# verdurin/pbdagcon

Measured on AMD Instinct MI355X. Metric: consensus bases/sec (whole node), higher is better.
Workload: dtype u8

## Files before the change

### pbdagcon_amd/csrc/k_build.hip.h

```cpp
#pragma once
#include <hip/hip_runtime.h>
#include "dagcon_dev.h"
#include "k_norm_run.hip.h"

#define DG_WAVE 64
#ifndef DG_LPW
#define DG_LPW 8u
#endif

__device__ __forceinline__ bool dg_failed(const DgParams &p) {
    return __hip_atomic_load(&p.st->err_flags, __ATOMIC_RELAXED, __HIP_MEMORY_SCOPE_AGENT) != 0;
}
__device__ __forceinline__ void dg_fail(const DgParams &p, uint32_t bit) {
    atomicOr(&p.st->err_flags, bit);
}
__device__ __forceinline__ void dg_fail_target(const DgParams &p, uint32_t t, uint32_t bit) {
    atomicOr(&p.tfail[t], bit);
}
__device__ __forceinline__ bool dg_tskip(const DgParams &p, uint32_t t) {
    return !p.tactive[t] || __hip_atomic_load(&p.tfail[t], __ATOMIC_RELAXED, __HIP_MEMORY_SCOPE_AGENT) != 0;
}
__device__ __forceinline__ bool dg_askip(const DgParams &p, uint32_t a) {
    return !(p.flags & DG_F_A1_ONLY) && __hip_atomic_load(&p.tfail[p.aln_tgt[a]], __ATOMIC_RELAXED, __HIP_MEMORY_SCOPE_AGENT) != 0;
}
__device__ __forceinline__ void dg_fail_aln(const DgParams &p, uint32_t a, uint32_t bit) {
    if (p.flags & DG_F_A1_ONLY) dg_fail(p, bit);
    else dg_fail_target(p, p.aln_tgt[a], bit);
    p.st->bad_aln = a;
}

#define DG_NW 64u
#define DG_NW_BIG 512u
#define DG_REDO 0xFFFFFFFFu

template <typename CT>
__device__ __forceinline__ void dg_store_run(const DgParams &p, CT *cell, const uint32_t run) {
    if constexpr (sizeof(CT) == 1) {
        if (run > 255u) { dg_fail(p, DG_E_RUN_WIDE); return; }
    }
    *cell = (CT)run;
}

template <typename CT>
__device__ inline void dg_finish_alignment(const DgParams &p, uint32_t a, uint16_t *buf, uint32_t m) {
    const uint32_t trim = p.trim;
    uint32_t lbases = 0, rbases = 0, lo = 0, hi = m;
    uint32_t start = p.aln_start[a];
    while (lbases < trim && lo < m) {
        if (DG_T(buf[lo++]) != DG_GAP) lbases++;
    }
    while (rbases < trim && hi > lo) {
        if (DG_T(buf[--hi]) != DG_GAP) rbases++;
    }
    start += lbases;
    const bool graph = !(p.flags & DG_F_A1_ONLY);
    uint32_t t_idx = 0, r = 0;
    CT *Cm = nullptr;
    if (graph) {
        t_idx = p.aln_tgt[a];
        if (p.tactive[t_idx]) {
            const uint64_t ab = p.aln_begin[t_idx];
            r = (uint32_t)(a - ab);
            Cm = static_cast<CT *>(p.matC) + p.matc_base[t_idx] + (uint64_t)r * p.matc_stride[t_idx];
        }
    }
    const uint32_t tlen = graph ? p.tlen[t_idx] : 0xFFFFFFFFu;
    uint32_t n_ins = 0, n_del = 0, adv = 0, run = 0;
    bool conf = start >= 1;
    uint32_t i = lo;
#define DG_FIN_COL(c, ci_)                                                                \
    do {                                                                                  \
        const uint8_t qb_ = DG_Q(c), tb_ = DG_T(c);                                       \
        if (qb_ == tb_ || qb_ == DG_GAP) {                                                \
            if (Cm && conf && ((start + adv) & ((1u << p.emit_shift) - 1u)) == 0 && start + adv <= tlen + 1) \
                ck[(start + adv) >> p.emit_shift] = ci_ - run;                            \
            if (run) { if (Cm && conf && start + adv <= tlen + 1) dg_store_run(p, Cm + (start + adv), run); run = 0; } \
            adv++; n_del += (qb_ != tb_);                                                 \
            if ((uint64_t)start - 1 + adv > (uint64_t)tlen) conf = false;                 \
        } else if (tb_ == DG_GAP) { n_ins++; run++; }                                     \
    } while (0)
    uint32_t *ck = p.ckpt + p.ck_base[a];
    while (i < hi && (i & 7u)) { const uint16_t c = buf[i]; DG_FIN_COL(c, i); i++; }
    while (i + 8 <= hi) {
        const uint4 v = *reinterpret_cast<const uint4 *>(buf + i);
        const uint32_t w4[4] = {v.x, v.y, v.z, v.w};
#pragma unroll
        for (int k = 0; k < 4; k++) {
            const uint16_t c0 = (uint16_t)(w4[k] & 0xffffu), c1 = (uint16_t)(w4[k] >> 16);
            DG_FIN_COL(c0, i + 2 * k);
            DG_FIN_COL(c1, i + 2 * k + 1);
        }
        i += 8;
    }
    while (i < hi) { const uint16_t c = buf[i]; DG_FIN_COL(c, i); i++; }
    if (run && Cm && conf && ((start + adv) & ((1u << p.emit_shift) - 1u)) == 0 && start + adv <= tlen + 1)
        ck[(start + adv) >> p.emit_shift] = hi - run;
    if (run && Cm && conf && start + adv <= tlen + 1) dg_store_run(p, Cm + (start + adv), run);
#undef DG_FIN_COL
    p.n_lo[a] = lo; p.n_hi[a] = hi; p.n_start[a] = start;
    p.n_ins[a] = n_ins; p.n_del[a] = n_del;
    atomicAdd(&p.st->n_columns, (unsigned long long)(hi - lo));
    if (graph && hi > lo && !conf) dg_fail_aln(p, a, DG_E_NONCONF);
}

template <uint32_t NW, uint32_t LANES, bool RETRY>
__global__ __launch_bounds__(LANES, RETRY ? 1 : 5) void k_norm_chunk(DgParams p) {
    __shared__ uint16_t s_win[LANES * (NW + 2u)];
    const uint32_t g = threadIdx.x * gridDim.x + blockIdx.x;
    if (g >= p.n_chunks) return;
    if (dg_failed(p)) return;
    if (RETRY && p.ch_flag[g] != 2u) return;
    const uint32_t a = p.ch_aln[g];
    if (dg_askip(p, a)) { if (!RETRY) p.ch_flag[g] = 0; return; }
    const uint32_t c = g - p.ch_base[a], nwin = p.ch_base[a + 1] - p.ch_base[a];
    const uint64_t off = p.aln_off[a];
    const uint32_t len = p.aln_len[a];
    const uint8_t *q = p.q + off, *t = p.t + off;
    uint32_t flag = 0;
    DgChunkRun r;
    r.w = 0; r.tb = 0; r.dirty = false; r.overflow = false; r.badchar = false;
    uint32_t k0 = DG_CH_NONE, cn = c + 1;
    uint64_t src = 0;
    if (p.flags & DG_F_RAW) {
        if (c == 0) { k0 = 0; cn = nwin; flag = 1; }
    } else {
        k0 = dg_chunk_start(q, t, len, c);
        if (k0 != DG_CH_NONE) {
            uint16_t *win = s_win + threadIdx.x * (NW + 2u);
            src = (2ull * (off + k0) + 8ull * g + 7ull) & ~7ull;
            for (;;) {
                uint32_t k1 = len;
                for (; cn < nwin; cn++) {
                    const uint32_t s = dg_chunk_start(q, t, len, cn);
                    if (s != DG_CH_NONE) { k1 = s; break; }
                }
                if constexpr (NW == DG_NW) r = dg_norm_run_gc(q, t, len, k0, k1, win, p.norm_tmp + src);
                else r = dg_norm_run<NW>(q, t, len, k0, k1, win, p.norm_tmp + src);
                if (r.badchar) dg_fail_aln(p, a, DG_E_BADCHAR);
                if (r.overflow) { flag = RETRY ? 1u : 2u; break; }
                if (!r.dirty) break;
                cn++;
                uint32_t k2 = len;
                for (uint32_t x = cn; x < nwin; x++) {
                    const uint32_t s = dg_chunk_start(q, t, len, x);
                    if (s != DG_CH_NONE) { k2 = s; break; }
                }
                const unsigned long long need = (2ull * (k2 - k0) + 15ull) & ~7ull;
                const unsigned long long o = atomicAdd(&p.st->ovf_top, need);
                if (p.tmp_main + o + need > p.tmp_cap) { flag = 1; break; }
                src = p.tmp_main + o;
            }
        }
    }
    p.ch_k0[g] = k0; p.ch_next[g] = cn; p.ch_w[g] = r.w; p.ch_tb[g] = r.tb;
    p.ch_flag[g] = flag; p.ch_src[g] = src;
}

__global__ __launch_bounds__(64) void k_norm_scan(DgParams p) {
    const uint32_t a = blockIdx.x * 64 + threadIdx.x;
    if (a >= p.A) return;
    if (dg_failed(p)) return;
    if (dg_askip(p, a)) return;
    const uint32_t g0 = p.ch_base[a], g1 = p.ch_base[a + 1];
    bool redo = false;
    uint32_t m = 0, tbt = 0;
    for (uint32_t g = g0; g < g1;) {
        if (p.ch_k0[g] == DG_CH_NONE) { p.ch_out[g] = DG_CH_NONE; g++; continue; }
        redo |= p.ch_flag[g] != 0;
        p.ch_out[g] = m; p.ch_adv[g] = tbt;
        m += p.ch_w[g]; tbt += p.ch_tb[g];
        uint32_t nx = g0 + p.ch_next[g];
        if (nx > g1) nx = g1;
        for (uint32_t x = g + 1; x < nx; x++) p.ch_out[x] = DG_CH_NONE;
        g = nx;
    }
    if (redo) { p.n_hi[a] = DG_REDO; return; }
    const uint32_t trim = p.trim;
    uint32_t lbases = 0, rbases = 0, lo = 0, hi = m;
    for (uint32_t g = g0; g < g1 && lbases < trim && lo < m; g++) {
        if (p.ch_out[g] == DG_CH_NONE) continue;
        const uint32_t w = p.ch_w[g], tb = p.ch_tb[g];
        if (lbases + tb < trim) { lo += w; lbases += tb; continue; }
        const uint16_t *src = p.norm_tmp + p.ch_src[g];
        for (uint32_t x = 0; x < w && lbases < trim; x++) {
            if (DG_T(src[x]) != DG_GAP) lbases++;
            lo++;
        }
    }
    for (uint32_t g = g1; g > g0 && rbases < trim && hi > lo;) {
        g--;
        const uint32_t o = p.ch_out[g];
        if (o == DG_CH_NONE) continue;
        const uint32_t tb = p.ch_tb[g];
        if (o >= lo && rbases + tb < trim) { hi = o; rbases += tb; continue; }
        const uint16_t *src = p.norm_tmp + p.ch_src[g];
        while (rbases < trim && hi > lo && hi > o) {
            if (DG_T(src[--hi - o]) != DG_GAP) rbases++;
        }
    }
    p.n_lo[a] = lo; p.n_hi[a] = hi; p.n_start[a] = p.aln_start[a] + lbases; p.n_lb[a] = lbases;
    p.n_ins[a] = 0; p.n_del[a] = 0;
    atomicAdd(&p.st->n_columns, (unsigned long long)(hi - lo));
}

__device__ __forceinline__ uint4 dg_funnel_cols(const uint4 A, const uint4 B, const uint32_t h) {
    const bool w1 = (h >> 1) & 1u, w2 = (h >> 2) & 1u, half = h & 1u;
    const uint32_t u0 = w1 ? A.y : A.x, u1 = w1 ? A.z : A.y, u2 = w1 ? A.w : A.z, u3 = w1 ? B.x : A.w,
                   u4 = w1 ? B.y : B.x, u5 = w1 ? B.z : B.y, u6 = w1 ? B.w : B.z;
    const uint32_t t0 = w2 ? u2 : u0, t1 = w2 ? u3 : u1, t2 = w2 ? u4 : u2, t3 = w2 ? u5 : u3, t4 = w2 ? u6 : u4;
    uint4 r;
    r.x = half ? __builtin_amdgcn_alignbit(t1, t0, 16) : t0;
    r.y = half ? __builtin_amdgcn_alignbit(t2, t1, 16) : t1;
    r.z = half ? __builtin_amdgcn_alignbit(t3, t2, 16) : t2;
    r.w = half ? __builtin_amdgcn_alignbit(t4, t3, 16) : t3;
    return r;
}

__device__ __forceinline__ uint32_t dg_wave_excl(const uint32_t v, const int lane) {
    int incl = (int)v;
    incl += __builtin_amdgcn_update_dpp(0, incl, 0x111, 0xf, 0xf, false);
    incl += __builtin_amdgcn_update_dpp(0, incl, 0x112, 0xf, 0xf, false);
    incl += __builtin_amdgcn_update_dpp(0, incl, 0x114, 0xf, 0xf, false);
    incl += __builtin_amdgcn_update_dpp(0, incl, 0x118, 0xf, 0xf, false);
    incl += __builtin_amdgcn_update_dpp(0, incl, 0x142, 0xa, 0xf, false);
    incl += __builtin_amdgcn_update_dpp(0, incl, 0x143, 0xc, 0xf, false);
    (void)lane;
    return (uint32_t)incl - v;
}

template <typename CT>
__global__ __launch_bounds__(256) void k_norm_finish2(DgParams p) {
    const uint32_t g = blockIdx.x * 4u + (threadIdx.x >> 6);
    if (g >= p.n_chunks) return;
    if (dg_failed(p)) return;
    const int lane = threadIdx.x & 63;
    const uint32_t a = p.ch_aln[g];
    if (dg_askip(p, a)) return;
    const uint32_t o = p.ch_out[g];
    if (o == DG_CH_NONE) return;
    const uint32_t hi = p.n_hi[a];
    if (hi == DG_REDO) return;
    const uint32_t lo = p.n_lo[a], start = p.n_start[a], lb = p.n_lb[a];
    const uint32_t w = p.ch_w[g], adv0 = p.ch_adv[g];
    const uint16_t *src = p.norm_tmp + p.ch_src[g];
    const uint4 *src4 = reinterpret_cast<const uint4 *>(src);
    uint16_t *dst = p.norm + p.norm_off[a] + o;
    const bool graph = !(p.flags & DG_F_A1_ONLY);
    uint32_t t_idx = 0;
    CT *Cm = nullptr;
    if (graph) {
        t_idx = p.aln_tgt[a];
        if (p.tactive[t_idx]) Cm = static_cast<CT *>(p.matC) + p.matc_base[t_idx] + (uint64_t)(a - p.aln_begin[t_idx]) * p.matc_stride[t_idx];
    }
    const uint32_t tlen = graph ? p.tlen[t_idx] : 0xFFFFFFFFu;
    uint32_t *ck = p.ckpt + p.ck_base[a];
    const uint32_t ck_mask = (1u << p.emit_shift) - 1u;
    const uint32_t adv_init = adv0 > lb ? adv0 - lb : 0u;
    const uint32_t f0 = lo > o ? lo - o : 0u;
    const uint32_t f1 = hi > o ? (hi - o < w ? hi - o : w) : 0u;
    const bool any = f1 > f0;
    const uint32_t fspan = any ? f1 - f0 : 0u;
#define DG_FIN_CONF(A) (start >= 1u && ((A) == 0u || (uint64_t)start - 1u + (A) <= (uint64_t)tlen))
    const uint32_t h0 = (8u - (o & 7u)) & 7u;
    const uint32_t h = h0 < w ? h0 : w;
    const uint32_t nb = (w - h) / 8u, nvec = (w + 7u) / 8u;
    if ((uint32_t)lane < h) dst[lane] = src[lane];
    { const uint32_t x = h + 8u * nb + (uint32_t)lane; if (lane < 8 && x < w) dst[x] = src[x]; }
    uint4 *dst4 = reinterpret_cast<uint4 *>(dst + h);
    uint32_t adv_tile = adv_init, run_tile = 0, n_ins = 0, n_del = 0;
    for (uint32_t v0 = 0; v0 < nvec; v0 += 64u) {
        const uint32_t vl = v0 + (uint32_t)lane;
        const uint4 pc = vl < nvec ? src4[vl] : make_uint4(0, 0, 0, 0);
        const uint4 pn = vl + 1 < nvec ? src4[vl + 1] : make_uint4(0, 0, 0, 0);
        if (vl < nb) dst4[vl] = dg_funnel_cols(pc, pn, h);
        if (!any || 8u * v0 >= f1) continue;
        uint32_t advm = 0, insm = 0, delm = 0;
#pragma unroll
        for (uint32_t k = 0; k < 8u; k++) {
            const uint32_t wd = ((k >> 1) & 3u) == 0 ? pc.x : ((k >> 1) & 3u) == 1 ? pc.y : ((k >> 1) & 3u) == 2 ? pc.z : pc.w;
            const uint16_t c = (uint16_t)((k & 1u) ? wd >> 16 : wd & 0xffffu);
            const bool inw = 8u * vl + k < 8u * nvec && 8u * vl + k - f0 < fspan;
            const uint8_t qb = DG_Q(c), tb = DG_T(c);
            const bool adv = inw && (qb == tb || qb == DG_GAP);
            advm |= adv ? 1u << k : 0u;
            delm |= (adv && qb != tb) ? 1u << k : 0u;
            insm |= (inw && !adv && tb == DG_GAP) ? 1u << k : 0u;
        }
        const uint32_t nadv = (uint32_t)__popc(advm), nI = (uint32_t)__popc(insm);
        n_ins += nI; n_del += (uint32_t)__popc(delm);
        const uint32_t adv_lane = adv_tile + dg_wave_excl(nadv, lane);
        uint32_t sf = advm ? 1u : 0u;
        uint32_t sv = advm ? (uint32_t)__popc(insm & ~((2u << (31 - __clz((int)advm))) - 1u)) : nI;
#pragma unroll
        for (int d = 1; d < 64; d <<= 1) {
            const uint32_t pf = (uint32_t)__shfl_up((int)sf, d), pv = (uint32_t)__shfl_up((int)sv, d);
            if (lane >= d) { sv = sf ? sv : pv + sv; sf |= pf; }
        }
        uint32_t ef = (uint32_t)__shfl_up((int)sf, 1), ev = (uint32_t)__shfl_up((int)sv, 1);
        if (lane == 0) { ef = 0; ev = 0; }
        uint32_t run = ef ? ev : ev + run_tile;
        const uint32_t lf = (uint32_t)__builtin_amdgcn_readlane((int)sf, 63), lv = (uint32_t)__builtin_amdgcn_readlane((int)sv, 63);
        run_tile = lf ? lv : lv + run_tile;
        adv_tile += (uint32_t)__builtin_amdgcn_readlane((int)(adv_lane - adv_tile + nadv), 63);
        uint32_t adv = adv_lane;
        if (Cm && (advm | insm)) {
#pragma unroll
            for (uint32_t k = 0; k < 8u; k++) {
                if ((advm >> k) & 1u) {
                    const bool conf = DG_FIN_CONF(adv);
                    const uint32_t x = 8u * vl + k;
                    if (conf && ((start + adv) & ck_mask) == 0 && start + adv <= tlen + 1 && !(x == 0 && o > lo))
                        ck[(start + adv) >> p.emit_shift] = o + x - run;
                    if (run && conf && start + adv <= tlen + 1) dg_store_run(p, Cm + (start + adv), run);
                    run = 0;
                    adv++;
                } else if ((insm >> k) & 1u) run++;
            }
        }
    }
    {
        const uint32_t adv = adv_tile, run = run_tile;
        const bool conf = DG_FIN_CONF(adv);
        if (lane == 0) {
            if (any && Cm && conf && ((start + adv) & ck_mask) == 0 && start + adv <= tlen + 1 && (o + f1 < hi || run))
                ck[(start + adv) >> p.emit_shift] = o + f1 - run;
            if (run && Cm && conf && start + adv <= tlen + 1) dg_store_run(p, Cm + (start + adv), run);
            if (graph && any && !conf) dg_fail_aln(p, a, DG_E_NONCONF);
        }
    }
    {
        const uint32_t ti = dg_wave_excl(n_ins, lane) + n_ins, td = dg_wave_excl(n_del, lane) + n_del;
        if (lane == 63) { if (ti) atomicAdd(&p.n_ins[a], ti); if (td) atomicAdd(&p.n_del[a], td); }
    }
#undef DG_FIN_CONF
}

template <typename CT>
__global__ __launch_bounds__(64) void k_normalize_slow(DgParams p) {
    const uint32_t a = blockIdx.x * 64 + threadIdx.x;
    if (a >= p.A) return;
    if (dg_failed(p)) return;
    if (dg_askip(p, a)) return;
    if (p.n_hi[a] != DG_REDO) return;
    const uint64_t off = p.aln_off[a];
    const uint32_t len = p.aln_len[a];
    const uint8_t *q = p.q + off, *t = p.t + off;
    uint16_t *buf = p.norm + p.norm_off[a];
    const bool raw = (p.flags & DG_F_RAW) != 0;
    uint32_t n = 0;
    for (uint32_t i = 0; i < len; i++) {
        uint8_t qb = q[i], tb = t[i];
        if (qb < 33 || qb > 126 || tb < 33 || tb > 126) dg_fail_aln(p, a, DG_E_BADCHAR);
        if (!raw) {
            if (qb == '.') qb = DG_GAP;
            if (tb == '.') tb = DG_GAP;
            if (qb != tb && qb != DG_GAP && tb != DG_GAP) {
                buf[n++] = DG_COL(DG_GAP, tb);
                buf[n++] = DG_COL(qb, DG_GAP);
                continue;
            }
        }
        buf[n++] = DG_COL(qb, tb);
    }
    uint32_t m = n;
    if (!raw) {
        uint32_t w = 0, jt = 0, jq = 0;
        for (uint32_t i = 0; i < n; i++) {
            uint16_t c = buf[i];
            uint8_t qi = DG_Q(c), ti = DG_T(c);
            if (i + 1 < n) {
                if (ti == DG_GAP) {
                    if (jt <= i) jt = i + 1;
                    while (jt < n && DG_T(buf[jt]) == DG_GAP) jt++;
                    if (jt < n) {
                        uint16_t cj = buf[jt];
                        if (DG_T(cj) == qi) { ti = qi; buf[jt] = DG_COL(DG_Q(cj), DG_GAP); }
                    }
                }
                if (qi == DG_GAP) {
                    if (jq <= i) jq = i + 1;
                    while (jq < n && DG_Q(buf[jq]) == DG_GAP) jq++;
                    if (jq < n) {
                        uint16_t cj = buf[jq];
                        if (DG_Q(cj) == ti) { qi = ti; buf[jq] = DG_COL(DG_GAP, DG_T(cj)); }
                    }
                }
            }
            if (qi != DG_GAP || ti != DG_GAP) buf[w++] = DG_COL(qi, ti);
        }
        m = w;
    }
    dg_finish_alignment<CT>(p, a, buf, m);
}

__device__ __forceinline__ uint32_t dg_pool_words(uint32_t tlen, uint32_t n_ins, uint32_t n_del,
                                                  uint32_t k, uint32_t growth_pct, uint32_t *fixed_words) {
    const uint64_t capb = dg_capb(k);
    const uint64_t fixed = 3ull * n_ins + (uint64_t)(tlen + 2) * 3ull * capb;
    const uint64_t spill = 3ull * ((uint64_t)n_ins + n_del + 2ull * k) + 64ull;
    const uint64_t growth = (fixed * growth_pct) / 100ull + spill + 256ull;
    *fixed_words = (uint32_t)fixed;
    const uint64_t tot = fixed + growth;
    return tot > 0xFFFFFFF0ull ? 0xFFFFFFF0u : (uint32_t)tot;
}

__global__ __launch_bounds__(1024) void k_carve(DgParams p) {
    __shared__ unsigned long long s_scan[1024];
    __shared__ unsigned long long s_carry_nodes, s_carry_pool;
    if (dg_failed(p)) return;
    const uint32_t tid = threadIdx.x;
    if (tid == 0) { s_carry_nodes = 0; s_carry_pool = 0; }
    __syncthreads();
    for (uint32_t t0 = 0; t0 < p.T; t0 += 1024) {
        const uint32_t t = t0 + tid;
        unsigned long long nodes = 0, poolw = 0;
        uint32_t fixed_words = 0, ins = 0;
        if (t < p.T && !dg_tskip(p, t)) {
            uint32_t del = 0;
            const uint64_t b = p.aln_begin[t], e = p.aln_begin[t + 1];
            for (uint64_t a = b; a < e; a++) { ins += p.n_ins[a]; del += p.n_del[a]; }
            nodes = (unsigned long long)p.tlen[t] + 2ull + ins;
            poolw = dg_pool_words(p.tlen[t], ins, del, (uint32_t)(e - b), p.growth_pct, &fixed_words);
            if (nodes > DG_MAX_NODES || poolw > 0x3FFFFFFFull) {
                dg_fail_target(p, t, DG_E_TOO_BIG);
                nodes = 0; poolw = 0; fixed_words = 0;
            }
        }
        s_scan[tid] = nodes;
        __syncthreads();
        for (uint32_t o = 1; o < 1024; o <<= 1) {
            unsigned long long v = tid >= o ? s_scan[tid - o] : 0;
            __syncthreads();
            s_scan[tid] += v;
            __syncthreads();
        }
        unsigned long long node_excl = s_scan[tid] - nodes + s_carry_nodes;
        unsigned long long node_tot = s_scan[1023];
        __syncthreads();
        s_scan[tid] = poolw;
        __syncthreads();
        for (uint32_t o = 1; o < 1024; o <<= 1) {
            unsigned long long v = tid >= o ? s_scan[tid - o] : 0;
            __syncthreads();
            s_scan[tid] += v;
            __syncthreads();
        }
        unsigned long long pool_excl = s_scan[tid] - poolw + s_carry_pool;
        unsigned long long pool_tot = s_scan[1023];
        __syncthreads();
        if (t < p.T) {
            p.node_base[t] = node_excl;
            p.n_nodes[t] = (uint32_t)nodes;
            p.pool_base[t] = pool_excl;
            p.pool_size[t] = (uint32_t)poolw;
            p.pool_top[t] = fixed_words;
            p.t_nins[t] = ins;
        }
        if (tid == 0) { s_carry_nodes += node_tot; s_carry_pool += pool_tot; }
        __syncthreads();
    }
    if (tid == 0) {
        p.st->node_need = s_carry_nodes;
        p.st->pool_need = s_carry_pool;
        if (s_carry_nodes > p.node_cap) dg_fail(p, DG_E_NODE_OVF);
        if (s_carry_pool > p.pool_cap) dg_fail(p, DG_E_POOL_OVF);
    }
}

__global__ __launch_bounds__(64) void k_readspan(DgParams p) {
    const uint32_t a = blockIdx.x * 64 + threadIdx.x;
    if (a >= p.A) return;
    if (dg_failed(p)) return;
    const uint32_t t = p.aln_tgt[a];
    uint32_t s = 0, e = 0, lead = 0, trail = 0;
    if (!dg_tskip(p, t)) {
        const uint32_t lo = p.n_lo[a], hi = p.n_hi[a];
        if (hi > lo && hi != DG_REDO) {
            const uint16_t *col = p.norm + p.norm_off[a];
            const uint32_t ins = p.n_ins[a];
            uint32_t i = lo, dels = 0;
            for (; i < hi; i++) {
                const uint8_t qb = DG_Q(col[i]), tb = DG_T(col[i]);
                if (qb == tb) break;
                if (tb == DG_GAP) lead++; else if (qb == DG_GAP) dels++;
            }
            s = p.n_start[a] + dels;
            if (i < hi) {
                uint32_t k = hi, tdels = 0;
                while (k > i + 1) {
                    const uint8_t qb = DG_Q(col[k - 1]), tb = DG_T(col[k - 1]);
                    if (qb == tb) break;
                    if (tb == DG_GAP) trail++; else if (qb == DG_GAP) tdels++;
                    k--;
                }
                e = p.n_start[a] + (hi - lo - ins) - 1u - tdels;
            } else { e = 0; s = 0; }
        }
    }
    p.rd_s[a] = s; p.rd_e[a] = e; p.rd_lead[a] = lead; p.rd_trail[a] = trail;
}

__global__ __launch_bounds__(256) void k_groups(DgParams p) {
    const uint32_t t = blockIdx.x;
    if (dg_failed(p) || dg_tskip(p, t)) return;
    const int lane = threadIdx.x & 63, wave = threadIdx.x >> 6;
    const uint32_t blen = p.tlen[t];
    const uint32_t K = (uint32_t)(p.aln_begin[t + 1] - p.aln_begin[t]);
    uint32_t *col0 = static_cast<uint32_t *>(p.matC) + p.matc_base[t];
    const uint32_t cstride = p.matc_stride[t];
    uint32_t *gcount = p.gcount + p.bbv_base[t];
    const uint32_t pos0 = (blockIdx.y * 4 + wave) * 8u;
    if (pos0 >= blen + 2) return;
    uint32_t carry[8];
#pragma unroll
    for (int j = 0; j < 8; j++) carry[j] = 0;
    for (uint32_t r0 = 0; r0 < K; r0 += DG_WAVE) {
        const uint32_t r = r0 + lane;
        uint4 *cell = reinterpret_cast<uint4 *>(col0 + (uint64_t)r * cstride + pos0);
        uint4 a = make_uint4(0, 0, 0, 0), b = a;
        if (r < K) { a = cell[0]; b = cell[1]; }
        uint32_t v[8] = {a.x, a.y, a.z, a.w, b.x, b.y, b.z, b.w};
        uint32_t ex[8];
#pragma unroll
        for (int j = 0; j < 8; j++) {
            uint32_t incl = v[j];
            for (int o = 1; o < DG_WAVE; o <<= 1) {
                const uint32_t up = __shfl_up(incl, o);
                if (lane >= o) incl += up;
            }
            ex[j] = carry[j] + incl - v[j];
            carry[j] += __shfl(incl, DG_WAVE - 1);
        }
        if (r < K) {
            cell[0] = make_uint4(ex[0], ex[1], ex[2], ex[3]);
            cell[1] = make_uint4(ex[4], ex[5], ex[6], ex[7]);
        }
    }
#pragma unroll
    for (int j = 0; j < 8; j++)
        if (lane == j && pos0 + j < blen + 2) gcount[pos0 + j] = carry[j];
}

__global__ __launch_bounds__(1024) void k_gscan(DgParams p) {
    __shared__ uint32_t s_scan[1024];
    __shared__ uint32_t s_carry;
    const uint32_t t = blockIdx.x;
    if (dg_failed(p) || dg_tskip(p, t)) return;
    const uint32_t tid = threadIdx.x;
    const uint32_t np = p.tlen[t] + 2;
    const uint64_t bv = p.bbv_base[t];
    if (tid == 0) s_carry = 0;
    __syncthreads();
    for (uint32_t p0 = 0; p0 < np; p0 += 1024) {
        const uint32_t pos = p0 + tid;
        const uint32_t gc = pos < np ? p.gcount[bv + pos] : 0u;
        const uint32_t v = pos < np ? gc + 1u : 0u;
        s_scan[tid] = v;
        __syncthreads();
        for (uint32_t o = 1; o < 1024; o <<= 1) {
            uint32_t x = tid >= o ? s_scan[tid - o] : 0;
            __syncthreads();
            s_scan[tid] += x;
            __syncthreads();
        }
        const uint32_t excl = s_scan[tid] - v + s_carry;
        const uint32_t tot = s_scan[1023];
        __syncthreads();
        if (pos < np) { p.gbase[bv + pos] = excl; p.bid[bv + pos] = excl + gc; }
        if (tid == 0) s_carry += tot;
        __syncthreads();
    }
    if (tid == 0 && s_carry != p.n_nodes[t]) dg_fail_target(p, t, DG_E_INTERNAL);
}

#define DG_CELL_DUP 0x1FFFFFEu
#define DG_EDONE 0xFFFFFFFFu
#define DG_EF_BB 1u
#define DG_EF_OWN 2u
__device__ __forceinline__ uint32_t dg_emit_fold(unsigned long long em, const uint32_t key, const uint32_t first, const uint32_t pos,
                                                 DgNode *ndt, uint32_t *pool, uint32_t *n_out, const int lane) {
    uint32_t victim = 0;
    *n_out = 0;
    while (em & (em - 1ull)) {
        const int f = __ffsll((long long)em) - 1;
        const uint32_t kf = (uint32_t)__builtin_amdgcn_readlane((int)key, f);
        const unsigned long long same = __ballot(key == kf);
        em &= ~same;
        const uint32_t n = (uint32_t)__popcll(same);
        if (n < 2 || !((same >> lane) & 1ull)) continue;
        const uint32_t nins = (key & 0xFF0000u) ? 3u : (key & 0xFF00u) ? 2u : 1u;
        if (lane == f) {
            *n_out = n;
            for (uint32_t k = 0; k < nins; k++) {
                const uint32_t id = first + k, rk = id - pos;
                reinterpret_cast<DgNode *>(reinterpret_cast<char *>(ndt) + (id << 5))->weight = (int32_t)n;
                pool[3u * rk + 1u] = n;
            }
        } else {
            victim = 1;
            for (uint32_t k = 0; k < nins; k++) {
                const uint32_t base = (key >> (8u * (nins - 1u - k))) & 0xFFu;
                *reinterpret_cast<uint2 *>(reinterpret_cast<char *>(ndt) + ((first + k) << 5)) = make_uint2(0u, base | (DG_NF_DELETED << 8));
            }
        }
    }
    return victim;
}

template <typename CT> struct DgGsum { static constexpr uint32_t PPT = sizeof(CT) == 1 ? 4u : 1u; };
template <typename CT>
__global__ __launch_bounds__(256) void k_gsum(DgParams p) {
    const uint32_t t = blockIdx.x;
    if (dg_failed(p) || dg_tskip(p, t)) return;
    const uint32_t pos = (blockIdx.y * 256u + threadIdx.x) * DgGsum<CT>::PPT;
    const uint32_t np = p.tlen[t] + 2u;
    if (pos >= np) return;
    const uint32_t K = (uint32_t)(p.aln_begin[t + 1] - p.aln_begin[t]);
    const CT *col = static_cast<const CT *>(p.matC) + p.matc_base[t] + pos;
    const uint32_t stride = p.matc_stride[t];
    uint32_t *gc = p.gcount + p.bbv_base[t] + pos;
    if constexpr (sizeof(CT) == 1) {
        uint32_t even = 0, odd = 0;
        for (uint32_t r = 0; r < K; r++) {
            const uint32_t w = *reinterpret_cast<const uint32_t *>(col + (uint64_t)r * stride);
            even += w & 0x00FF00FFu; odd += (w >> 8) & 0x00FF00FFu;
        }
        const uint32_t s[4] = {even & 0xFFFFu, odd & 0xFFFFu, even >> 16, odd >> 16};
        if (pos + 3u < np) *reinterpret_cast<uint4 *>(gc) = make_uint4(s[0], s[1], s[2], s[3]);
        else for (uint32_t j = 0; pos + j < np; j++) gc[j] = s[j];
    } else {
        uint32_t sum = 0;
        for (uint32_t r = 0; r < K; r++) sum += col[(uint64_t)r * stride];
        *gc = sum;
    }
}

#ifndef DG_EB
// ... 638 lines not shown
```

Before: 364.8 million.

## Rework normalize-finish kernel with multi-vector lanes, SWAR masks, and DPP segmented scan

Each lane in k_norm_finish2 now handles DG_FIN_NP uint4 vectors instead of one. Per-column classification becomes SWAR byte compares that build advance, insert and delete masks. The shfl_up segmented run-length scan is replaced by a DPP-based segmented scan. Run stores and checkpoint writes are visited sparsely by iterating set bits under a ballot loop instead of looping over all 8 columns, cutting per-column branching and shuffle cost. The added helper logic risks subtle correctness errors and adds register pressure.

```diff
diff --git a/pbdagcon_amd/csrc/k_build.hip.h b/pbdagcon_amd/csrc/k_build.hip.h
--- a/pbdagcon_amd/csrc/k_build.hip.h
+++ b/pbdagcon_amd/csrc/k_build.hip.h
@@ -2,6 +2,7 @@
 #include <hip/hip_runtime.h>
 #include "dagcon_dev.h"
 #include "k_norm_run.hip.h"
+#include "k_norm_fin.hip.h"
 
 #define DG_WAVE 64
 #ifndef DG_LPW
@@ -228,9 +229,21 @@
     return (uint32_t)incl - v;
 }
 
+__device__ __forceinline__ uint32_t dg_wave_seg_incl(uint32_t x) {
+#define DG_SEG_STEP(CTRL, ROWS) x = dg_seg_combine((uint32_t)__builtin_amdgcn_update_dpp(0, (int)x, CTRL, ROWS, 0xf, false), x)
+    DG_SEG_STEP(0x111, 0xf);
+    DG_SEG_STEP(0x112, 0xf);
+    DG_SEG_STEP(0x114, 0xf);
+    DG_SEG_STEP(0x118, 0xf);
+    DG_SEG_STEP(0x142, 0xa);
+    DG_SEG_STEP(0x143, 0xc);
+#undef DG_SEG_STEP
+    return x;
+}
+
 template <typename CT>
 __global__ __launch_bounds__(256) void k_norm_finish2(DgParams p) {
-    const uint32_t g = blockIdx.x * 4u + (threadIdx.x >> 6);
+    const uint32_t g = blockIdx.x * 4u + (uint32_t)__builtin_amdgcn_readfirstlane((int)(threadIdx.x >> 6));
     if (g >= p.n_chunks) return;
     if (dg_failed(p)) return;
     const int lane = threadIdx.x & 63;
@@ -254,13 +267,11 @@
     }
     const uint32_t tlen = graph ? p.tlen[t_idx] : 0xFFFFFFFFu;
     uint32_t *ck = p.ckpt + p.ck_base[a];
-    const uint32_t ck_mask = (1u << p.emit_shift) - 1u;
+    const DgFinChunk u = dg_fin_chunk(start, tlen, p.emit_shift, o, lo);
     const uint32_t adv_init = adv0 > lb ? adv0 - lb : 0u;
     const uint32_t f0 = lo > o ? lo - o : 0u;
     const uint32_t f1 = hi > o ? (hi - o < w ? hi - o : w) : 0u;
     const bool any = f1 > f0;
-    const uint32_t fspan = any ? f1 - f0 : 0u;
-#define DG_FIN_CONF(A) (start >= 1u && ((A) == 0u || (uint64_t)start - 1u + (A) <= (uint64_t)tlen))
     const uint32_t h0 = (8u - (o & 7u)) & 7u;
     const uint32_t h = h0 < w ? h0 : w;
     const uint32_t nb = (w - h) / 8u, nvec = (w + 7u) / 8u;
@@ -268,61 +279,59 @@
     { const uint32_t x = h + 8u * nb + (uint32_t)lane; if (lane < 8 && x < w) dst[x] = src[x]; }
     uint4 *dst4 = reinterpret_cast<uint4 *>(dst + h);
     uint32_t adv_tile = adv_init, run_tile = 0, n_ins = 0, n_del = 0;
-    for (uint32_t v0 = 0; v0 < nvec; v0 += 64u) {
-        const uint32_t vl = v0 + (uint32_t)lane;
-        const uint4 pc = vl < nvec ? src4[vl] : make_uint4(0, 0, 0, 0);
-        const uint4 pn = vl + 1 < nvec ? src4[vl + 1] : make_uint4(0, 0, 0, 0);
-        if (vl < nb) dst4[vl] = dg_funnel_cols(pc, pn, h);
+    const bool writes = Cm != nullptr && u.ok;
+    for (uint32_t v0 = 0; v0 < nvec; v0 += 64u * DG_FIN_NP) {
+        const uint32_t vl = v0 + DG_FIN_NP * (uint32_t)lane;
+        uint4 pc[DG_FIN_NP + 1u];
+#pragma unroll
+        for (uint32_t j = 0; j <= DG_FIN_NP; j++) pc[j] = src4[vl + j < nvec ? vl + j : nvec - 1u];
+#pragma unroll
+        for (uint32_t j = 0; j < DG_FIN_NP; j++)
+            if (vl + j < nb) dst4[vl + j] = dg_funnel_cols(pc[j], pc[j + 1u], h);
         if (!any || 8u * v0 >= f1) continue;
         uint32_t advm = 0, insm = 0, delm = 0;
 #pragma unroll
-        for (uint32_t k = 0; k < 8u; k++) {
-            const uint32_t wd = ((k >> 1) & 3u) == 0 ? pc.x : ((k >> 1) & 3u) == 1 ? pc.y : ((k >> 1) & 3u) == 2 ? pc.z : pc.w;
-            const uint16_t c = (uint16_t)((k & 1u) ? wd >> 16 : wd & 0xffffu);
-            const bool inw = 8u * vl + k < 8u * nvec && 8u * vl + k - f0 < fspan;
-            const uint8_t qb = DG_Q(c), tb = DG_T(c);
-            const bool adv = inw && (qb == tb || qb == DG_GAP);
-            advm |= adv ? 1u << k : 0u;
-            delm |= (adv && qb != tb) ? 1u << k : 0u;
-            insm |= (inw && !adv && tb == DG_GAP) ? 1u << k : 0u;
-        }
-        const uint32_t nadv = (uint32_t)__popc(advm), nI = (uint32_t)__popc(insm);
-        n_ins += nI; n_del += (uint32_t)__popc(delm);
-        const uint32_t adv_lane = adv_tile + dg_wave_excl(nadv, lane);
-        uint32_t sf = advm ? 1u : 0u;
-        uint32_t sv = advm ? (uint32_t)__popc(insm & ~((2u << (31 - __clz((int)advm))) - 1u)) : nI;
-#pragma unroll
-        for (int d = 1; d < 64; d <<= 1) {
-            const uint32_t pf = (uint32_t)__shfl_up((int)sf, d), pv = (uint32_t)__shfl_up((int)sv, d);
-            if (lane >= d) { sv = sf ? sv : pv + sv; sf |= pf; }
-        }
-        uint32_t ef = (uint32_t)__shfl_up((int)sf, 1), ev = (uint32_t)__shfl_up((int)sv, 1);
-        if (lane == 0) { ef = 0; ev = 0; }
-        uint32_t run = ef ? ev : ev + run_tile;
-        const uint32_t lf = (uint32_t)__builtin_amdgcn_readlane((int)sf, 63), lv = (uint32_t)__builtin_amdgcn_readlane((int)sv, 63);
-        run_tile = lf ? lv : lv + run_tile;
-        adv_tile += (uint32_t)__builtin_amdgcn_readlane((int)(adv_lane - adv_tile + nadv), 63);
-        uint32_t adv = adv_lane;
-        if (Cm && (advm | insm)) {
-#pragma unroll
-            for (uint32_t k = 0; k < 8u; k++) {
-                if ((advm >> k) & 1u) {
-                    const bool conf = DG_FIN_CONF(adv);
-                    const uint32_t x = 8u * vl + k;
-                    if (conf && ((start + adv) & ck_mask) == 0 && start + adv <= tlen + 1 && !(x == 0 && o > lo))
-                        ck[(start + adv) >> p.emit_shift] = o + x - run;
-                    if (run && conf && start + adv <= tlen + 1) dg_store_run(p, Cm + (start + adv), run);
-                    run = 0;
-                    adv++;
-                } else if ((insm >> k) & 1u) run++;
+        for (uint32_t j = 0; j < DG_FIN_NP; j++) {
+            const DgFinMasks m = dg_fin_piece(pc[j]);
+            advm |= m.advm << (8u * j); insm |= m.insm << (8u * j); delm |= m.delm << (8u * j);
+        }
+        const uint32_t win = dg_fin_window(8u * vl, f0, f1);
+        advm &= win; insm &= win; delm &= win;
+        const uint32_t nadv = (uint32_t)__popc(advm);
+        n_ins += (uint32_t)__popc(insm); n_del += (uint32_t)__popc(delm);
+        const uint32_t adv_rel = dg_wave_excl(nadv, lane);
+        const uint32_t adv_lane = adv_tile + adv_rel;
+        const uint32_t seg = dg_wave_seg_incl(dg_seg_pack(advm, insm));
+        const uint32_t seg_front = (uint32_t)__builtin_amdgcn_update_dpp(0, (int)seg, 0x138, 0xf, 0xf, false);
+        const uint32_t run_in = dg_seg_value(dg_seg_combine(run_tile, seg_front));
+        run_tile = dg_seg_value(dg_seg_combine(run_tile, (uint32_t)__builtin_amdgcn_readlane((int)seg, 63)));
+        adv_tile += (uint32_t)__builtin_amdgcn_readlane((int)(adv_rel + nadv), 63);
+        if (!writes) continue;
+        uint32_t ends = dg_fin_run_ends(advm, insm, run_in);
+        while (__ballot(ends != 0u)) {
+            if (ends) {
+                const uint32_t k = (uint32_t)__builtin_ctz(ends);
+                ends &= ends - 1u;
+                const DgFinEvent e = dg_fin_event(u, advm, insm, run_in, adv_lane, k);
+                if (e.writes) dg_store_run(p, Cm + e.pos, e.run);
+            }
+        }
+        uint32_t jc = dg_fin_first_ckpt(u, adv_lane);
+        while (__ballot(jc < nadv)) {
+            if (jc < nadv) {
+                const uint32_t k = dg_fin_nth_adv(advm, jc);
+                const DgFinEvent e = dg_fin_event(u, advm, insm, run_in, adv_lane, k);
+                uint32_t slot, value;
+                if (dg_fin_ckpt(u, e, 8u * vl + k, slot, value)) ck[slot] = value;
+                jc += u.ck_mask + 1u;
             }
         }
     }
     {
         const uint32_t adv = adv_tile, run = run_tile;
-        const bool conf = DG_FIN_CONF(adv);
+        const bool conf = dg_fin_conf(u, adv);
         if (lane == 0) {
-            if (any && Cm && conf && ((start + adv) & ck_mask) == 0 && start + adv <= tlen + 1 && (o + f1 < hi || run))
+            if (any && Cm && conf && ((start + adv) & u.ck_mask) == 0 && start + adv <= tlen + 1 && (o + f1 < hi || run))
                 ck[(start + adv) >> p.emit_shift] = o + f1 - run;
             if (run && Cm && conf && start + adv <= tlen + 1) dg_store_run(p, Cm + (start + adv), run);
             if (graph && any && !conf) dg_fail_aln(p, a, DG_E_NONCONF);
@@ -332,7 +341,6 @@
         const uint32_t ti = dg_wave_excl(n_ins, lane) + n_ins, td = dg_wave_excl(n_del, lane) + n_del;
         if (lane == 63) { if (ti) atomicAdd(&p.n_ins[a], ti); if (td) atomicAdd(&p.n_del[a], td); }
     }
-#undef DG_FIN_CONF
 }
 
 template <typename CT>
diff --git a/pbdagcon_amd/csrc/k_norm_fin.hip.h b/pbdagcon_amd/csrc/k_norm_fin.hip.h
--- /dev/null
+++ b/pbdagcon_amd/csrc/k_norm_fin.hip.h
@@ -0,0 +1,100 @@
+#pragma once
+#include "k_norm_run.hip.h"
+
+#ifndef DG_FIN_NP
+#define DG_FIN_NP 2u
+#endif
+#define DG_FIN_COLS (8u * DG_FIN_NP)
+#define DG_FIN_ALL ((1u << DG_FIN_COLS) - 1u)
+
+DG_HD_INLINE void dg_fin_word(const uint32_t w, uint32_t &K, uint32_t &D) {
+    const uint32_t G = dg_eq_bytes(w, 0x2D2D2D2Du);
+    const uint32_t E = dg_eq_bytes(w, w >> 8);
+    const uint32_t A = (E | G) & 0x00800080u;
+    const uint32_t I = ~A & (G >> 8) & 0x00800080u;
+    K = A | (I << 8);
+    D = A & ~E;
+}
+
+struct DgFinMasks { uint32_t advm, insm, delm; };
+
+DG_HD_INLINE DgFinMasks dg_fin_piece(const dg_u4 pc) {
+    uint32_t K0, K1, K2, K3, D0, D1, D2, D3;
+    dg_fin_word(pc.x, K0, D0); dg_fin_word(pc.y, K1, D1); dg_fin_word(pc.z, K2, D2); dg_fin_word(pc.w, K3, D3);
+    uint32_t k = (K0 >> 7) | (K1 >> 5) | (K2 >> 3) | (K3 >> 1);
+    uint32_t d = (D0 >> 7) | (D1 >> 5) | (D2 >> 3) | (D3 >> 1);
+    k |= k >> 15; d |= d >> 15;
+    DgFinMasks m;
+    m.advm = k & 0xFFu; m.insm = (k >> 8) & 0xFFu; m.delm = d & 0xFFu;
+    return m;
+}
+
+DG_HD_INLINE uint32_t dg_fin_window(const uint32_t c0, const uint32_t f0, const uint32_t f1) {
+    const uint32_t a = f0 > c0 ? (f0 - c0 < DG_FIN_COLS ? f0 - c0 : DG_FIN_COLS) : 0u;
+    const uint32_t b = f1 > c0 ? (f1 - c0 < DG_FIN_COLS ? f1 - c0 : DG_FIN_COLS) : 0u;
+    return b > a ? ((1u << b) - 1u) & ~((1u << a) - 1u) : 0u;
+}
+
+#define DG_SEG_RESET 0x80000000u
+DG_HD_INLINE uint32_t dg_seg_pack(const uint32_t advm, const uint32_t insm) {
+    if (!advm) return (uint32_t)__builtin_popcount(insm);
+    const uint32_t upto = (2u << (31 - __builtin_clz(advm))) - 1u;
+    return DG_SEG_RESET | (uint32_t)__builtin_popcount(insm & ~upto);
+}
+DG_HD_INLINE uint32_t dg_seg_combine(const uint32_t a, const uint32_t b) { return (b & DG_SEG_RESET) ? b : a + b; }
+DG_HD_INLINE uint32_t dg_seg_value(const uint32_t x) { return x & ~DG_SEG_RESET; }
+
+DG_HD_INLINE uint32_t dg_fin_run_ends(const uint32_t advm, const uint32_t insm, const uint32_t run_in) {
+    const uint32_t a = advm << 1, b = (insm << 1) | (run_in ? 1u : 0u);
+    return (a & ~(a - b)) >> 1;
+}
+
+DG_HD_INLINE uint32_t dg_fin_run_at(const uint32_t advm, const uint32_t insm, const uint32_t run_in, const uint32_t k) {
+    const uint32_t below = (1u << k) - 1u, prev = advm & below;
+    const uint32_t behind = ~0u << (31 - __builtin_clz((prev << 1) | 1u));
+    return (prev ? 0u : run_in) + (uint32_t)__builtin_popcount(insm & below & behind);
+}
+
+DG_HD_INLINE uint32_t dg_fin_nth_adv(uint32_t advm, uint32_t j) {
+    while (j--) advm &= advm - 1u;
+    return (uint32_t)__builtin_ctz(advm);
+}
+
+struct DgFinChunk {
+    uint32_t start, tlen, lim, ck_mask, ck_shift;
+    uint32_t o, lo;
+    bool ok;
+};
+DG_HD_INLINE DgFinChunk dg_fin_chunk(const uint32_t start, const uint32_t tlen, const uint32_t emit_shift, const uint32_t o,
+                                     const uint32_t lo) {
+    DgFinChunk u;
+    u.start = start; u.tlen = tlen; u.ck_shift = emit_shift; u.ck_mask = (1u << emit_shift) - 1u; u.o = o; u.lo = lo;
+    u.ok = start >= 1u;
+    const uint64_t room = (uint64_t)tlen + 1u;
+    u.lim = !u.ok ? 0u : room >= start ? (uint32_t)(room - start) : 0u;
+    return u;
+}
+DG_HD_INLINE bool dg_fin_conf(const DgFinChunk &u, const uint32_t adv) { return u.ok && adv <= u.lim; }
+DG_HD_INLINE bool dg_fin_writes(const DgFinChunk &u, const uint32_t adv) {
+    return dg_fin_conf(u, adv) && u.start + adv <= u.tlen + 1u;
+}
+
+struct DgFinEvent { uint32_t pos, run; bool writes; };
+DG_HD_INLINE DgFinEvent dg_fin_event(const DgFinChunk &u, const uint32_t advm, const uint32_t insm, const uint32_t run_in,
+                                     const uint32_t adv_lane, const uint32_t k) {
+    DgFinEvent e;
+    const uint32_t adv = adv_lane + (uint32_t)__builtin_popcount(advm & ((1u << k) - 1u));
+    e.pos = u.start + adv;
+    e.run = dg_fin_run_at(advm, insm, run_in, k);
+    e.writes = dg_fin_writes(u, adv);
+    return e;
+}
+
+DG_HD_INLINE uint32_t dg_fin_first_ckpt(const DgFinChunk &u, const uint32_t adv_lane) {
+    return (0u - (u.start + adv_lane)) & u.ck_mask;
+}
+DG_HD_INLINE bool dg_fin_ckpt(const DgFinChunk &u, const DgFinEvent &e, const uint32_t x, uint32_t &slot, uint32_t &value) {
+    slot = e.pos >> u.ck_shift;
+    value = u.o + x - e.run;
+    return e.writes && !(x == 0u && u.o > u.lo);
+}
```

Measured after the change: 376.2 million (median of 6 runs). 3.1% higher.
